# mims-harvard/SubGNN

Hardware: AMD Instinct MI355X
Metric: subgraphs/sec fwd+bwd (all 3 channels on) + achieved HBM GB/s (higher is better)
Workload: dtype f32; 1 GPU; synthetic DENSITY-style BA base graph n=1000000 m=10 (9998512 undirected edges), 50000 BFS subgraphs x 20 nodes per GPU (weak form; BASELINE configs[3] "50k sharded across 8" as worded is --scaling strong), all_density hparams (N 10/43, P 57/183, S 42, 1 layer), D=64, full pass = sampling + similarities + fwd + bwd + Adam; subgraphs_per_gpu=50000, subgraphs_total=50000

## Files before the change

### include/subgnn_hip.h

```cpp
#ifndef SUBGNN_HIP_H
#define SUBGNN_HIP_H

#include <stdint.h>

#ifdef __cplusplus
extern "C" {
#endif

#define SGNN_OK                  0
#define SGNN_ERR_BAD_ARG        -1
#define SGNN_ERR_SET_TOO_LARGE  -2
#define SGNN_ERR_NNZ_TOO_LARGE  -3
#define SGNN_ERR_LAUNCH         -4
#define SGNN_ERR_UNSUPPORTED_D  -5

#define SGNN_ABI_VERSION 12
int sgnn_abi_version(void);
int sgnn_warm_up(void* stream);
const char* sgnn_last_error(void);

int sgnn_degree_sequence(const int64_t* rowptr, const int32_t* col, int64_t nnz,
                         const int32_t* full_degree, const uint8_t* self_loops,
                         const int64_t* set_ptr, const int32_t* set_nodes, int64_t n_sets,
                         int64_t max_set_size, int sorted,
// ... 103 lines not shown
                          void* stream);
int sgnn_triangular_walks_both(const int64_t* rowptr, const int32_t* col, const int32_t* col_sorted, int64_t nnz,
                               const int64_t* patch_ptr, const int32_t* patch_nodes, const int64_t* inb_ptr,
                               const int32_t* inb_nodes, int64_t n_items, int64_t walks_per_patch, int64_t walk_len,
                               double beta, uint64_t seed, uint64_t stream_id_int, uint64_t stream_id_bor,
                               int64_t item_base, int64_t max_id, int64_t* out, void* stream);

int sgnn_patch_in_border(const int64_t* rowptr, const int32_t* col, int64_t nnz,
                         const int32_t* node_order, const int32_t* node_pos, int64_t n_nodes,
                         const int64_t* patch_ptr, const int32_t* patch_nodes, int64_t n_patches,
                         uint8_t* out_flag, void* stream);
int64_t sgnn_patch_in_border_huge_workspace_bytes(int64_t total_nodes);
int sgnn_patch_in_border_huge(const int64_t* rowptr, const int32_t* col, int64_t nnz,
                              const int32_t* node_order, const int32_t* node_pos, int64_t n_nodes,
                              const int64_t* patch_ptr, const int32_t* patch_nodes, int64_t n_patches,
                              int64_t total_nodes, uint8_t* out_flag, void* workspace, int64_t workspace_bytes,
                              void* stream);

int sgnn_sp_similarity_dense(const double* apsp, int64_t n_cols,
                             const int64_t* set_ptr, const int32_t* set_nodes, int64_t n_sets,
                             float* out, void* stream);
int64_t sgnn_bfs_hops_workspace_bytes(int64_t max_id, int64_t n_sources, int max_hops);
int sgnn_bfs_hops(const int64_t* rowptr, const int32_t* col, int64_t nnz, int64_t max_id,
                  const int32_t* sources, int64_t n_sources, int max_hops, int node_major, int pull_alpha,
                  uint8_t* dist, void* workspace, int64_t workspace_bytes, void* stream);
int sgnn_min_hops_to_sets(const uint8_t* dist, int64_t n_sources, int64_t max_id, int node_major,
                          const int64_t* set_ptr, const int32_t* set_nodes, int64_t n_sets,
                          float* out, void* stream);
int64_t sgnn_bfs_min_hops_workspace_bytes(int64_t max_id, int64_t n_sources, int max_hops, int64_t n_sets);
int sgnn_bfs_min_hops_to_sets(const int64_t* rowptr, const int32_t* col, int64_t nnz, int64_t max_id,
                              const int32_t* sources, int64_t n_sources, int max_hops, int pull_alpha, int push_levels,
                              const int64_t* set_ptr, const int32_t* set_nodes, int64_t n_sets,
                              float* out, int32_t* out_status, void* workspace, int64_t workspace_bytes, void* stream);

int sgnn_dtw_order_keys(const int64_t* x_ptr, const int32_t* x_val, int64_t n_x, int64_t* out_keys, void* stream);
int64_t sgnn_dtw_workspace_bytes(int64_t n_x, int64_t max_x_len, int64_t n_y, int64_t max_y_len);
int sgnn_dtw_similarity(const int64_t* x_ptr, const int32_t* x_val, int64_t n_x, int64_t max_x_len,
                        const int64_t* y_ptr, const int32_t* y_val, int64_t n_y, int64_t max_y_len,
                        int tie_order, int kernel, const int32_t* x_order, float* out, void* workspace,
                        int64_t workspace_bytes, void* stream);
int sgnn_dtw_similarity_live(const int64_t* x_ptr, const int32_t* x_val, int64_t n_x, int64_t max_x_len,
                             const int64_t* y_ptr, const int32_t* y_val, int64_t n_y, int64_t max_y_len,
                             int tie_order, int kernel, const int32_t* x_order, const int64_t* x_live_range, float* out,
                             void* workspace, int64_t workspace_bytes, void* stream);

int64_t sgnn_dtw_exact_workspace_bytes(int64_t n_x, int64_t max_x_len, int64_t n_y, int64_t max_y_len);
int sgnn_dtw_exact_similarity(const int64_t* x_ptr, const int32_t* x_val, int64_t n_x, int64_t max_x_len,
                              const int64_t* y_ptr, const int32_t* y_val, int64_t n_y, int64_t max_y_len,
                              int kernel, const int32_t* x_order, float* out, void* workspace,
                              int64_t workspace_bytes, void* stream);
int sgnn_dtw_exact_similarity_live(const int64_t* x_ptr, const int32_t* x_val, int64_t n_x, int64_t max_x_len,
                                   const int64_t* y_ptr, const int32_t* y_val, int64_t n_y, int64_t max_y_len,
                                   int kernel, const int32_t* x_order, const int64_t* x_live_range, float* out,
                                   void* workspace, int64_t workspace_bytes, void* stream);

int sgnn_cc_embed_fwd(const float* E, int64_t D,
                      const int64_t* set_ptr, const int32_t* set_nodes, int64_t n_sets,
                      int aggregator, int64_t padded_len, float* out, int32_t* out_arg, void* stream);
int sgnn_cc_embed_fwd_f16(const uint16_t* E_half, int64_t D,
                          const int64_t* set_ptr, const int32_t* set_nodes, int64_t n_sets,
                          int aggregator, int64_t padded_len, float* out, int32_t* out_arg, void* stream);
int sgnn_cc_embed_bwd(const float* grad_out, int64_t D,
                      const int64_t* set_ptr, const int32_t* set_nodes, int64_t n_sets,
                      int aggregator, const int32_t* arg, float* grad_E, void* stream);

#define SGNN_SRC_DENSE  0
// ... 219 lines not shown
```

### subgnn_amd/_lib.py

```python
import ctypes
import os

_HERE = os.path.dirname(os.path.abspath(__file__))
LIB_PATH = os.path.join(_HERE, 'lib', 'libsubgnn_hip.so')

c_i64 = ctypes.c_int64
c_u64 = ctypes.c_uint64
c_int = ctypes.c_int
c_dbl = ctypes.c_double
c_ptr = ctypes.c_void_p


class MpnArgs(ctypes.Structure):
    _fields_ = [('src', ctypes.c_int32), ('sims_per_edge', ctypes.c_int32),
                ('R', c_i64), ('A', c_i64), ('D', c_i64),
                ('x', c_ptr), ('ids', c_ptr), ('id_div', c_i64), ('edge_mask', c_ptr), ('row_mask', c_ptr),
                ('sims', c_ptr), ('sims_ld', c_i64), ('sim_col', c_ptr), ('wp', c_ptr), ('bp', c_ptr),
                ('x_f16', ctypes.c_int32), ('z_act', c_ptr), ('flags', ctypes.c_int32)]


SIGNATURES = {
    'sgnn_abi_version': (c_int, []),
    'sgnn_warm_up': (c_int, [c_ptr]),
    'sgnn_last_error': (ctypes.c_char_p, []),
# ... 15 lines not shown
    'sgnn_cc_compact_huge': (c_int, [c_ptr, c_ptr, c_ptr, c_i64, c_i64, c_int, c_i64, c_i64, c_ptr, c_ptr, c_ptr, c_ptr, c_i64, c_ptr]),
    'sgnn_subgraph_properties_workspace_bytes': (c_i64, [c_i64]),
    'sgnn_subgraph_properties': (c_int, [c_ptr, c_ptr, c_i64, c_i64, c_int, c_ptr, c_ptr, c_i64, c_i64, c_i64, c_ptr, c_ptr, c_ptr, c_i64,
                                         c_ptr]),
    'sgnn_patch_in_border_huge_workspace_bytes': (c_i64, [c_i64]),
    'sgnn_patch_in_border_huge': (c_int, [c_ptr, c_ptr, c_i64, c_ptr, c_ptr, c_i64, c_ptr, c_ptr, c_i64, c_i64, c_ptr, c_ptr, c_i64, c_ptr]),
    'sgnn_sort_sets': (c_int, [c_ptr, c_ptr, c_i64, c_i64, c_ptr, c_ptr, c_ptr]),
    'sgnn_khop_border_workspace_bytes': (c_i64, [c_i64, c_i64, c_int]),
    'sgnn_khop_border_bitmap_fits_lds': (c_int, [c_i64]),
    'sgnn_khop_border': (c_int, [c_ptr, c_ptr, c_i64, c_i64, c_ptr, c_ptr, c_i64, c_int, c_int, c_ptr, c_ptr, c_ptr,
                                 c_ptr, c_ptr, c_i64, c_int, c_ptr]),
    'sgnn_khop_border_arena': (c_int, [c_ptr, c_ptr, c_i64, c_i64, c_ptr, c_ptr, c_i64, c_int, c_ptr, c_ptr, c_ptr, c_ptr,
                                       c_i64, c_int, c_ptr]),
    'sgnn_khop_border_sample_workspace_bytes': (c_i64, [c_i64, c_i64, c_int, c_int, c_int]),
    'sgnn_khop_border_sample': (c_int, [c_ptr, c_ptr, c_ptr, c_i64, c_i64, c_ptr, c_ptr, c_i64, c_int, c_i64, c_u64, c_u64, c_i64,
                                        c_ptr, c_ptr, c_ptr, c_ptr, c_ptr, c_ptr, c_i64, c_int, c_ptr]),
    'sgnn_khop1_border_sorted': (c_int, [c_ptr, c_ptr, c_ptr, c_i64, c_i64, c_ptr, c_ptr, c_i64, c_ptr, c_ptr, c_ptr, c_ptr, c_i64,
                                         c_int, c_ptr]),
    'sgnn_sample_border_anchors': (c_int, [c_ptr, c_ptr, c_ptr, c_i64, c_ptr, c_i64, c_u64, c_u64, c_i64, c_int, c_ptr, c_ptr,
                                           c_ptr]),
    'sgnn_sample_anchors_padded': (c_int, [c_ptr, c_i64, c_i64, c_i64, c_u64, c_u64, c_ptr, c_ptr]),
    'sgnn_sample_anchors_ragged': (c_int, [c_ptr, c_ptr, c_i64, c_ptr, c_i64, c_u64, c_u64, c_i64, c_ptr, c_ptr]),
    'sgnn_choice_ragged': (c_int, [c_ptr, c_ptr, c_i64, c_i64, c_u64, c_u64, c_i64, c_ptr, c_ptr]),
    'sgnn_triangular_walks_both': (c_int, [c_ptr, c_ptr, c_ptr, c_i64, c_ptr, c_ptr, c_ptr, c_ptr, c_i64, c_i64, c_i64, c_dbl, c_u64,
                                           c_u64, c_u64, c_i64, c_i64, c_ptr, c_ptr]),
    'sgnn_triangular_walks': (c_int, [c_ptr, c_ptr, c_ptr, c_i64, c_ptr, c_i64, c_ptr, c_ptr, c_ptr, c_ptr, c_int,
                                      c_i64, c_i64, c_i64, c_dbl, c_u64, c_u64, c_i64, c_i64, c_int, c_ptr, c_ptr]),
    'sgnn_patch_in_border': (c_int, [c_ptr, c_ptr, c_i64, c_ptr, c_ptr, c_i64, c_ptr, c_ptr, c_i64, c_ptr, c_ptr]),
    'sgnn_sp_similarity_dense': (c_int, [c_ptr, c_i64, c_ptr, c_ptr, c_i64, c_ptr, c_ptr]),
    'sgnn_bfs_hops_workspace_bytes': (c_i64, [c_i64, c_i64, c_int]),
    'sgnn_bfs_min_hops_workspace_bytes': (c_i64, [c_i64, c_i64, c_int, c_i64]),
    'sgnn_bfs_min_hops_to_sets': (c_int, [c_ptr, c_ptr, c_i64, c_i64, c_ptr, c_i64, c_int, c_int, c_int, c_ptr, c_ptr, c_i64, c_ptr, c_ptr,
                                          c_ptr, c_i64, c_ptr]),
    'sgnn_bfs_hops': (c_int, [c_ptr, c_ptr, c_i64, c_i64, c_ptr, c_i64, c_int, c_int, c_int, c_ptr, c_ptr, c_i64, c_ptr]),
    'sgnn_min_hops_to_sets': (c_int, [c_ptr, c_i64, c_i64, c_int, c_ptr, c_ptr, c_i64, c_ptr, c_ptr]),
    'sgnn_dtw_workspace_bytes': (c_i64, [c_i64, c_i64, c_i64, c_i64]),
    'sgnn_dtw_similarity': (c_int, [c_ptr, c_ptr, c_i64, c_i64, c_ptr, c_ptr, c_i64, c_i64, c_int, c_int, c_ptr, c_ptr, c_ptr,
                                    c_i64, c_ptr]),
    'sgnn_dtw_order_keys': (c_int, [c_ptr, c_ptr, c_i64, c_ptr, c_ptr]),
    'sgnn_dtw_similarity_live': (c_int, [c_ptr, c_ptr, c_i64, c_i64, c_ptr, c_ptr, c_i64, c_i64, c_int, c_int, c_ptr, c_ptr, c_ptr,
                                         c_ptr, c_i64, c_ptr]),
    'sgnn_dtw_exact_workspace_bytes': (c_i64, [c_i64, c_i64, c_i64, c_i64]),
    'sgnn_dtw_exact_similarity': (c_int, [c_ptr, c_ptr, c_i64, c_i64, c_ptr, c_ptr, c_i64, c_i64, c_int, c_ptr, c_ptr, c_ptr,
                                          c_i64, c_ptr]),
    'sgnn_dtw_exact_similarity_live': (c_int, [c_ptr, c_ptr, c_i64, c_i64, c_ptr, c_ptr, c_i64, c_i64, c_int, c_ptr, c_ptr, c_ptr,
                                               c_ptr, c_i64, c_ptr]),
    'sgnn_cc_embed_fwd': (c_int, [c_ptr, c_i64, c_ptr, c_ptr, c_i64, c_int, c_i64, c_ptr, c_ptr, c_ptr]),
    'sgnn_cc_embed_bwd': (c_int, [c_ptr, c_i64, c_ptr, c_ptr, c_i64, c_int, c_ptr, c_ptr, c_ptr]),
    'sgnn_mpn_fwd_chunks': (c_int, [ctypes.POINTER(MpnArgs)]),
    'sgnn_mpn_fwd': (c_int, [ctypes.POINTER(MpnArgs), c_ptr, c_ptr, c_ptr]),
    'sgnn_mpn_fwd_many_max_bodies': (c_i64, []),
    'sgnn_mpn_fwd_many': (c_int, [c_i64, c_ptr, c_ptr, c_ptr, c_ptr]),
    'sgnn_mpn_bwd': (c_int, [ctypes.POINTER(MpnArgs), c_ptr, c_ptr, c_ptr, c_ptr, c_ptr]),
    'sgnn_attn_scores_epilogue': (c_int, [c_ptr, c_ptr, c_ptr, c_i64, c_i64, c_i64, c_ptr, c_ptr]),
    'sgnn_attn_scores_f16_workspace_bytes': (c_i64, [c_i64]),
    'sgnn_attn_scores_fwd_f16': (c_int, [c_ptr, c_ptr, c_ptr, c_ptr, c_i64, c_i64, c_i64, c_ptr, c_ptr, c_i64, c_ptr]),
    'sgnn_lstm_supported': (c_int, [c_i64]),
    'sgnn_lstm_fwd': (c_int, [c_ptr, c_ptr, c_ptr, c_ptr, c_ptr, c_i64, c_i64, c_i64, c_ptr, c_ptr, c_ptr, c_ptr, c_ptr]),
    'sgnn_lstm_bwd': (c_int, [c_ptr, c_ptr, c_ptr, c_ptr, c_ptr, c_i64, c_i64, c_i64, c_ptr, c_ptr]),
    'sgnn_masked_sum_fwd': (c_int, [c_ptr, c_ptr, c_i64, c_i64, c_i64, c_ptr, c_ptr]),
    'sgnn_masked_sum_bwd': (c_int, [c_ptr, c_ptr, c_i64, c_i64, c_i64, c_ptr, c_ptr]),
    'sgnn_masked_sum_slot_fwd': (c_int, [c_ptr, c_ptr, c_i64, c_i64, c_i64, c_ptr, c_i64, c_ptr]),
    'sgnn_masked_sum_slot_bwd': (c_int, [c_ptr, c_i64, c_ptr, c_i64, c_i64, c_i64, c_ptr, c_ptr]),
    'sgnn_masked_sum_slots_fwd': (c_int, [c_ptr, c_ptr, c_ptr, c_i64, c_ptr, c_i64, c_i64, c_ptr, c_i64, c_ptr]),
    'sgnn_masked_sum_slots_bwd': (c_int, [c_ptr, c_i64, c_ptr, c_i64, c_i64, c_ptr, c_ptr, c_ptr, c_i64, c_ptr]),
    'sgnn_readout_sum_fwd': (c_int, [c_ptr, c_i64, c_ptr, c_ptr, c_ptr, c_ptr, c_i64, c_i64, c_i64, c_ptr, c_i64, c_ptr]),
# ... 126 lines not shown
```

### subgnn_amd/csrc/similarity.hip

```cpp
#include "common.h"
#include <type_traits>

__global__ __launch_bounds__(256) void sp_similarity_dense_kernel(
    const double* __restrict__ apsp, int64_t n_cols,
    const int64_t* __restrict__ set_ptr, const int32_t* __restrict__ set_nodes,
    float* __restrict__ out)
{
    const int64_t r = blockIdx.y;
    const int64_t beg = set_ptr[r];
    const int n = (int)(set_ptr[r + 1] - beg);
    for (int64_t c = blockIdx.x * (int64_t)blockDim.x + threadIdx.x; c < n_cols; c += (int64_t)gridDim.x * blockDim.x) {
        float res = 0.f;
        if (n > 0) {
            double m = apsp[(int64_t)(set_nodes[beg] - 1) * n_cols + c];
            for (int i = 1; i < n; ++i) {
                const double v = apsp[(int64_t)(set_nodes[beg + i] - 1) * n_cols + c];
                m = v < m ? v : m;
            }
            res = (float)m;
        }
        out[r * n_cols + c] = res;
    }
}

// ... 528 lines not shown
    for (int l = 2; l <= last_level && flags[l - 1] != 0; ++l) {
        bool pl, ppl;
        int kk;
        msbfs_mode(fvol, pull_above, push_levels, l, pl, ppl, kk);
        n_written += pl ? 1 : 0;
    }
    const uint64_t* lcur = pull ? B[(k + 1) % 3] : frontier;
    const uint64_t* lold = pull ? B[k % 3] : nullptr;
    for (int64_t t = blockIdx.x * (int64_t)blockDim.x + threadIdx.x; t < total; t += (int64_t)gridDim.x * blockDim.x) {
        if (reduce_last)
            msbfs_set_reduce_item(lcur, n_words, n_sources, set_ptr, set_nodes, set_seen, out, last_level, rs, t, lold);
        const int64_t r = t / n_words, w = t % n_words;
        uint64_t all = ~0ull;
        for (int64_t i = set_ptr[r]; i < set_ptr[r + 1]; ++i) {
            const int64_t v = set_nodes[i];
            if (!fdone[v]) all &= B[n_written % 3][v * rs + w];
        }
        uint64_t missing = ~all;
        while (missing) {
            const int b = __ffsll((unsigned long long)missing) - 1;
            missing &= missing - 1;
            const int64_t s = w * 64 + b;
            if (s < n_sources) out[r * n_sources + s] = 0.f;
        }
    }
}

__global__ void msbfs_status_kernel(const int32_t* __restrict__ flags, int max_hops, int32_t* __restrict__ status,
                                    const unsigned long long* __restrict__ fvol, unsigned long long pull_above, int push_levels)
{
    if (threadIdx.x == 0 && blockIdx.x == 0) msbfs_write_status(flags, fvol, pull_above, push_levels, max_hops, status);
}

static int msbfs_run(const int64_t* rowptr, const int32_t* col, int64_t nnz, int64_t max_id,
                     const int32_t* sources, int64_t n_sources, int max_hops, int node_major, uint8_t* dist,
                     const int64_t* set_ptr, const int32_t* set_nodes, int64_t n_sets, float* set_out,
                     void* workspace, hipStream_t st, int pull_alpha, int32_t* status = nullptr, int push_levels = -1)
{
    if (push_levels < 0 || pull_alpha == 0 || push_levels > max_hops) push_levels = max_hops;
    if (push_levels < 1) push_levels = 1;
    const int g_bfs_alpha = pull_alpha < 0 ? MSBFS_DEFAULT_ALPHA : pull_alpha;
    const int64_t n_ids = max_id + 1;
    const int64_t n_words = (n_sources + 63) / 64;
    const int64_t ss = node_major ? 1 : n_ids, sv = node_major ? n_sources : 1;
    const int64_t rs = msbfs_row_stride(n_words);
    uint64_t* seen = (uint64_t*)workspace;
    uint64_t* frontier = seen + n_ids * rs;
    uint64_t* next = frontier + n_ids * rs;
    unsigned long long* fvol = (unsigned long long*)(next + n_ids * rs);
    int32_t* flags = (int32_t*)(fvol + max_hops + 2);
    uint32_t* fbits = (uint32_t*)(((uintptr_t)(flags + max_hops + 2) + 7) & ~(uintptr_t)7);
    const int64_t fwords = (n_ids + 31) / 32;
    uint8_t* fdone = (uint8_t*)(fbits + 2 * fwords);
    uint64_t* set_seen = (uint64_t*)(((uintptr_t)(fbits + 2 * fwords + (n_ids + 3) / 4) + 7) & ~(uintptr_t)7);
    const unsigned long long pull_above =
        g_bfs_alpha > 0 ? (unsigned long long)((nnz * n_words) / g_bfs_alpha) : ~0ull;
    const int big = sgnn_grid_for(n_ids * ((dist && n_sources > rs) ? n_sources : rs), 256);
    hipLaunchKernelGGL(msbfs_init_kernel, dim3(big), dim3(256), 0, st, sources, n_sources, n_words, n_ids, seen,
                       frontier, next, dist, flags, fvol, fbits, max_hops, rs, set_seen, set_out ? n_sets * n_words : 0,
                       set_out, set_out ? n_sets * n_sources : 0);
    SGNN_CHECK_LAUNCH();
    hipLaunchKernelGGL(msbfs_seed_kernel, dim3((int)((n_sources + 255) / 256)), dim3(256), 0, st, sources, n_sources,
                       n_words, n_ids, seen, frontier, dist, ss, sv, fbits, rs);
    SGNN_CHECK_LAUNCH();
    const int g_sets = set_out ? sgnn_grid_for(n_sets * n_words, 256) : 0;
    MsbfsSets sets;
    sets.set_ptr = set_ptr; sets.set_nodes = set_nodes; sets.n_sets = set_out ? n_sets : 0; sets.set_seen = set_seen; sets.out = set_out;
    const int g_expand = sgnn_grid_for(n_ids * 16, 256);
    const int g_commit = sgnn_grid_for(n_ids, 256, 256 * 4);
    MsbfsBufs bufs;
    bufs.b[0] = seen; bufs.b[1] = next; bufs.b[2] = frontier;
    for (int level = 1; level <= max_hops; ++level) {
        hipLaunchKernelGGL(msbfs_level_kernel, dim3(g_expand), dim3(256), 0, st, rowptr, col, n_ids, n_words, n_sources,
                           bufs, flags, fvol, pull_above, push_levels, level, fbits, fbits + fwords, fdone, rs, sets, dist, ss, sv);
        SGNN_CHECK_LAUNCH();
        if (level <= push_levels) {
            hipLaunchKernelGGL(msbfs_commit_kernel, dim3(g_commit), dim3(256), 0, st, rowptr, n_ids, n_words, n_sources, seen,
                               frontier, next, dist, flags, fvol, level, ss, sv, fbits, fdone, rs, pull_above, push_levels);
            SGNN_CHECK_LAUNCH();
        }
    }
    if (set_out) {
        hipLaunchKernelGGL(msbfs_set_finalize_kernel, dim3(g_sets), dim3(256), 0, st, seen, n_words, n_sources, set_ptr,
                           set_nodes, n_sets, set_out, rs, frontier, set_seen, flags, max_hops, status, next, fvol, pull_above,
                           push_levels, fdone);
        SGNN_CHECK_LAUNCH();
    }
    if (status && !set_out) {
        hipLaunchKernelGGL(msbfs_status_kernel, dim3(1), dim3(64), 0, st, flags, max_hops, status, fvol, pull_above, push_levels);
        SGNN_CHECK_LAUNCH();
    }
    return SGNN_OK;
}

extern "C" int sgnn_bfs_hops(const int64_t* rowptr, const int32_t* col, int64_t nnz, int64_t max_id,
                             const int32_t* sources, int64_t n_sources, int max_hops, int node_major, int pull_alpha,
                             uint8_t* dist, void* workspace, int64_t workspace_bytes, void* stream)
{
    if (!rowptr || !col || !sources || !dist || !workspace || n_sources < 0 || max_hops < 1 || max_hops > 254)
        return SGNN_ERR_BAD_ARG;
    if (nnz >= (1ll << 31)) return SGNN_ERR_NNZ_TOO_LARGE;
    if (workspace_bytes < sgnn_bfs_hops_workspace_bytes(max_id, n_sources, max_hops)) return SGNN_ERR_BAD_ARG;
    if (n_sources == 0) return SGNN_OK;
    return msbfs_run(rowptr, col, nnz, max_id, sources, n_sources, max_hops, node_major, dist, nullptr, nullptr, 0,
                     nullptr, workspace, (hipStream_t)stream, pull_alpha);
}

extern "C" int64_t sgnn_bfs_min_hops_workspace_bytes(int64_t max_id, int64_t n_sources, int max_hops, int64_t n_sets) {
    const int64_t n_words = (n_sources + 63) / 64;
    return sgnn_bfs_hops_workspace_bytes(max_id, n_sources, max_hops) + 16 + n_sets * n_words * 8;
}

extern "C" int sgnn_bfs_min_hops_to_sets(const int64_t* rowptr, const int32_t* col, int64_t nnz, int64_t max_id,
                                         const int32_t* sources, int64_t n_sources, int max_hops, int pull_alpha, int push_levels,
                                         const int64_t* set_ptr, const int32_t* set_nodes, int64_t n_sets,
                                         float* out, int32_t* out_status, void* workspace, int64_t workspace_bytes,
                                         void* stream)
{
    if (!rowptr || !col || !sources || !set_ptr || !set_nodes || !out || !workspace || n_sources < 0 || n_sets < 0 ||
        max_hops < 1 || max_hops > 254)
        return SGNN_ERR_BAD_ARG;
    if (nnz >= (1ll << 31)) return SGNN_ERR_NNZ_TOO_LARGE;
    if (workspace_bytes < sgnn_bfs_min_hops_workspace_bytes(max_id, n_sources, max_hops, n_sets)) return SGNN_ERR_BAD_ARG;
    if (n_sources == 0 || n_sets == 0) return SGNN_OK;
    return msbfs_run(rowptr, col, nnz, max_id, sources, n_sources, max_hops, 0, nullptr, set_ptr, set_nodes, n_sets, out,
                     workspace, (hipStream_t)stream, pull_alpha, out_status, push_levels);
}

__global__ void min_hops_to_sets_kernel(const uint8_t* __restrict__ dist, int64_t n_sources, int64_t n_ids,
                                        const int64_t* __restrict__ set_ptr, const int32_t* __restrict__ set_nodes,
                                        int64_t n_sets, float* __restrict__ out, int64_t ss, int64_t sv)
{
    const int64_t total = n_sets * n_sources;
    for (int64_t t = blockIdx.x * (int64_t)blockDim.x + threadIdx.x; t < total; t += (int64_t)gridDim.x * blockDim.x) {
        const int64_t r = t / n_sources, a = t % n_sources;
        const int64_t beg = set_ptr[r];
        const int n = (int)(set_ptr[r + 1] - beg);
        int m = 0;
        for (int i = 0; i < n; ++i) {
            int d = dist[a * ss + (int64_t)set_nodes[beg + i] * sv];
            if (d == 255) d = 0;
            m = (i == 0 || d < m) ? d : m;
        }
        out[t] = (float)m;
    }
}

extern "C" int sgnn_min_hops_to_sets(const uint8_t* dist, int64_t n_sources, int64_t max_id, int node_major,
                                     const int64_t* set_ptr, const int32_t* set_nodes, int64_t n_sets,
                                     float* out, void* stream)
{
    if (!dist || !set_ptr || !set_nodes || !out || n_sources < 0 || n_sets < 0) return SGNN_ERR_BAD_ARG;
    if (n_sets * n_sources == 0) return SGNN_OK;
    hipLaunchKernelGGL(min_hops_to_sets_kernel, dim3(sgnn_grid_for(n_sets * n_sources, 256)), dim3(256), 0,
                       (hipStream_t)stream, dist, n_sources, max_id + 1, set_ptr, set_nodes, n_sets, out,
                       node_major ? 1 : max_id + 1, node_major ? n_sources : 1);
    SGNN_CHECK_LAUNCH();
    return SGNN_OK;
}
// ... 3 lines not shown
```

### subgnn_amd/hotpath.py

```python
import time

import collections

import torch

from . import ops, tape, gamma, subgraph_utils
from .graph_step import record, recording_key
from . import anchor_patch_samplers as aps

MAX_PINT_BYTES = 16 << 30


class StageTimer:

    def __init__(self, enabled=True):
        self.enabled, self.marks, self.host = enabled, [], []

    def mark(self, name):
        if self.enabled:
            e = torch.cuda.Event(enable_timing=True)
            e.record()
            self.marks.append((name, e))
            self.host.append(time.perf_counter())

# ... 7 lines not shown
        return out


def _hand_over(stream, *objs):
    for o in objs:
        if o is None:
            continue
        if isinstance(o, torch.Tensor):
            if o.is_cuda:
                o.record_stream(stream)
            for nm in ('_sgnn_ids32', '_sgnn_sorted', '_sgnn_both', '_sgnn_all', '_sgnn_mask', '_sgnn_mask_u8'):
                extra = getattr(o, nm, None)
                if extra is not None:
                    _hand_over(stream, extra)
        elif isinstance(o, ops.Ragged):
            _hand_over(stream, o.ptr, o.nodes)
        elif isinstance(o, dict):
            _hand_over(stream, *o.values())
        elif isinstance(o, (list, tuple)):
            _hand_over(stream, *o)


BFS_LEVEL_MARGIN = 2
WALKS_ON_SIDE_MAX_SETS = 16384


def _bfs_levels(model, key, max_hops):
    hint = model.__dict__.setdefault('_bfs_level_hint', {})
    k = hint.get(key)
    return max_hops if k is None else min(max_hops, k + BFS_LEVEL_MARGIN + 1)


BFS_PUSH_MARGIN = 1


def _bfs_push_levels(model, key):
    k = model.__dict__.setdefault('_bfs_push_hint', {}).get(key)
    return -1 if not k else int(k) - 1 + BFS_PUSH_MARGIN


def _bfs_note(model, st, key, status, max_hops, enqueued, redo):
    hint = model.__dict__.setdefault('_bfs_level_hint', {})
    if torch.cuda.is_current_stream_capturing():
        if hint.get(key) is None:
            raise RuntimeError('a recorded pass needs the BFS depth of an earlier eager pass (GraphedPasses warms up first)')
        pool = model.__dict__.setdefault('_bfs_status_pool', [])
        if not pool:
            raise RuntimeError('no pinned status buffer left for a recorded search: GraphedPasses._record provides them')
        host = pool.pop()
        host.copy_(status, non_blocking=True)
        st.bfs_checks.append((key, host, None, max_hops, enqueued, None))
        return
    if hint.get(key) is None:
        last, more, first_pull = status.tolist()[:3]
        model.__dict__.setdefault('_bfs_push_hint', {})[key] = first_pull
        if more:
            raise RuntimeError('position-channel BFS: level %d still reached new nodes -- hparams["max_bfs_hops"] = %d '
                               'is smaller than the depth of this graph from the anchors' % (max_hops, max_hops))
        hint[key] = last
        return
    pool = model.__dict__.setdefault('_bfs_status_pool', [])
    host = pool.pop() if pool else torch.empty(4, dtype=torch.int32).pin_memory()
    host.copy_(status, non_blocking=True)
    ev = torch.cuda.Event()
    ev.record(torch.cuda.current_stream())
    st.bfs_checks.append((key, host, ev, max_hops, enqueued, redo))
# ... 202 lines not shown
    sims = {}
    a_sets = ai = ae = None
    det = bool(getattr(model, '_deterministic', ops.DETERMINISTIC))
    side.wait_stream(main)
    with torch.cuda.stream(side):
        new_patches = hp['use_structure'] and pool is None and (split != 'test' or getattr(model, 'structure_anchors', None) is None)
        structure_anchors = getattr(model, 'structure_anchors', None) if pool is None else pool['structure_anchors']
        if new_patches:
            if shard is not None and shard.deal_shared and hp['structure_patch_type'] == 'triangular_random_walk':
                n_p = hp['max_sim_epochs'] * hp['n_anchor_patches_structure'] * hp['n_layers']
                structure_anchors = _deal_rows(shard, n_p, lambda lo, hi: aps.sample_structure_anchor_patches(
                    hp, g, dev, hp['max_sim_epochs'], trim=False, share=(lo, hi)), (hp['sample_walk_len'],), torch.int64, dev,
                    key=('S_patches', split))
                st.attrs['structure_anchors'] = structure_anchors
            else:
                structure_anchors = st.attrs['structure_anchors'] = aps.sample_structure_anchor_patches(hp, g, dev, hp['max_sim_epochs'], trim=False)
            if side is main:
                t.mark('S_patches_walks')
        patch_ev = None
        if hp['use_structure'] and side is not main:
            patch_ev = torch.cuda.Event()
            patch_ev.record(side)
        def position_block():
            if hp['use_position']:
                anchors_pos_ext = getattr(model, 'anchors_pos_ext', None)
                if anchors_pos_ext is None or split != 'test':
                    anchors_pos_ext = st.attrs['anchors_pos_ext'] = aps.init_anchors_pos_ext(hp, g, dev, epoch=ep)
                    if det:
                        for v in anchors_pos_ext.values():
                            ops.presort_ids(v, g.max_id)
                pint = {l: ops.choice_ragged(subs, hp['n_anchor_patches_pos_in'], seed,
                                             tape.stream_id(tape.STREAM_P_INT, split, l, ep), item_base=base) for l in range(L)}
                st.per_split['anchors_pos_int'] = pint
                for l in range(L):
                    if shard is not None and shard.deal_shared:
                        cap = hp.get('max_bfs_hops', 32)
                        if getattr(shard, 'emulator', None) is not None:
                            w, status = _emulated_position_sims(g, anchors_pos_ext[l], cc_sets, cc_ids, shard, cap, (split, l))
                        else:
                            w, status = _dealt_position_sims(g, anchors_pos_ext[l], cc_sets, cc_ids, shard, cap)
                        w = w.view(S, C, -1)
                        model.__dict__.setdefault('_bfs_level_hint', {}).setdefault(('P_out_dealt', split, l), 0)
                        _bfs_note(model, st, ('P_out_dealt', split, l), status, cap, cap, None)
                    else:
                        cap = hp.get('max_bfs_hops', 32)
                        nlev = _bfs_levels(model, ('P_out', split, l), cap)
                        src = anchors_pos_ext[l].to(torch.int32).contiguous()
                        w, status = ops.bfs_min_hops_to_sets(g, src, cc_sets, max_hops=nlev, want_status=True,
                                                             push_levels=_bfs_push_levels(model, ('P_out', split, l)))

                        def redo(levels, src=src, l=l, sims=sims):
                            _hand_over(torch.cuda.current_stream(), src, cc_sets)
                            w2, st2 = ops.bfs_min_hops_to_sets(g, src, cc_sets, max_hops=levels, want_status=True)
                            sims[('P', 'out', l)] = w2.view(S, C, -1).contiguous()
                            return st2.tolist()
                        _bfs_note(model, st, ('P_out', split, l), status, cap, nlev, redo)
                        w = w.view(S, C, -1)
                    sims[('P', 'out', l)] = w.contiguous()
                    if C == 1:
                        sims[('P', 'in', l)] = ops.ZeroSims((S, C, hp['n_anchor_patches_pos_in']), dev)
                    else:
                        uniq, inv = torch.unique(pint[l], return_inverse=True)
                        if uniq.numel() * (g.max_id + 1) <= MAX_PINT_BYTES:
                            d = ops.bfs_hops(g, uniq.to(torch.int32).contiguous(), max_hops=hp.get('max_bfs_hops', 32),
                                             node_major=True)
                            full = ops.min_hops_to_sets(d, cc_sets, node_major=True).view(S, C, -1)
                            w = torch.gather(full, 2, inv.view(S, 1, -1).expand(S, C, -1))
                        else:
                            w = _pint_sims_streamed(g, uniq, inv, cc_sets, S, C, hp.get('max_bfs_hops', 32))
                        sims[('P', 'in', l)] = (w * real.unsqueeze(-1)).contiguous()
                if side is main:
                    t.mark('P_bfs_sims')
        late_bfs = bool(hp.get('bfs_beside_dtw', False)) and side is not main and hp['use_structure'] and hp['use_position'] \
            and not defer_dtw and not (shard is not None and shard.deal_shared)
        wos = hp.get('walks_on_side_stream')
        walks_on_side = (bool(wos) if wos is not None else cc_sets.n <= WALKS_ON_SIDE_MAX_SETS) and side is not main and hp['use_structure']

        def structure_walks(degree_sequences=True):
            nonlocal a_sets, ai, ae
            if new_patches and shard is not None and shard.deal_shared:
                W_, T_ = hp['n_triangular_walks'], hp['random_walk_len']

                def both(lo, hi):
                    mine = structure_anchors[lo:hi].contiguous()
                    v = aps.patch_node_views(mine)
                    iw, bw = aps.perform_random_walks_both(hp, g, mine, v, first_patch=lo)
# ... 528 lines not shown
```

### subgnn_amd/ops.py

```python
import collections
import ctypes
import functools
import threading

import numpy as np
import torch

from . import _lib
from ._lib import MpnArgs, check

PAD = 0


def _ptr(t):
    return None if t is None else ctypes.c_void_p(t.data_ptr())


_RAW_STREAM = getattr(torch._C, '_cuda_getCurrentRawStream', None)
_CUR_DEVICE = getattr(torch._C, '_cuda_getDevice', None)


def _stream():
    if _RAW_STREAM is not None and _CUR_DEVICE is not None:
        return ctypes.c_void_p(_RAW_STREAM(_CUR_DEVICE()))
# ... 199 lines not shown
            hubs = torch.nonzero(deg >= thr).view(-1)
            H = int(hubs.numel())
            W, rows_n = (H + 31) // 32, self.max_id + 1
            if 0 < H and rows_n * W * 4 <= self.HUB_BITMAP_BYTES:
                dev = self.device
                hub_index = torch.full((self.max_id + 1,), -1, dtype=torch.int32, device=dev)
                hub_index[hubs] = torch.arange(H, dtype=torch.int32, device=dev)
                hdeg = deg[hubs]
                owner = torch.repeat_interleave(torch.arange(H, dtype=torch.int64, device=dev), hdeg)
                start = torch.cumsum(hdeg, 0) - hdeg
                pos = torch.arange(owner.numel(), dtype=torch.int64, device=dev) - start[owner] + self.rowptr[hubs][owner]
                x = self.col_sorted[pos].to(torch.int64)
                words = torch.zeros(rows_n * W, dtype=torch.int64, device=dev)
                words.index_add_(0, x * W + (owner >> 5), torch.ones_like(owner) << (owner & 31))
                out = (hub_index, words.to(torch.int32).view(rows_n, W).contiguous(), W)
        self.__dict__['_hub_tables'] = out
        return out

    def node_records(self):
        cached = self.__dict__.get('_node_records', False)
        if cached is not False:
            return cached
        out = None
        hub = self.hub_tables()
        if hub is not None:
            deg = (self.rowptr[1:] - self.rowptr[:-1]).to(torch.int32)
            sl = self.self_loops.to(torch.int32)
            z = ((sl.to(torch.int64) << 24) | torch.where(hub[0] >= 0, hub[0], torch.full_like(hub[0], 0xffffff)).to(torch.int64)).to(torch.int32)
            full = self.full_degree if self.full_degree is not None else deg + sl
            out = torch.stack([self.rowptr[:-1].to(torch.int32), deg, z, full.to(torch.int32)], 1).contiguous()
        self.__dict__['_node_records'] = out
        return out


_WARM = set()


def warm_up(device=None):
    if not torch.cuda.is_available():
        return 0.0
    dev = torch.device('cuda', torch.cuda.current_device()) if device is None else torch.device(device)
    if dev.type != 'cuda' or str(dev) in _WARM:
        return 0.0
    import time
    t0 = time.perf_counter()
    _WARM.add(str(dev))
    with torch.cuda.device(dev), torch.random.fork_rng(devices=[dev]):
        check(_lib.load().sgnn_warm_up(_stream()), 'sgnn_warm_up')
        i64 = torch.arange(8, device=dev)
        i32 = i64.to(torch.int32)
        f32 = torch.rand(8, 8, device=dev, requires_grad=True)
        torch.cumsum(i64, 0); torch.sort(i64); torch.argsort(i32); i64.index_select(0, i64 % 4); i64.max(); (i64 != 0).sum()
        torch.zeros(9, dtype=torch.int64, device=dev).scatter_(0, i64, i64); torch.where(i64 > 3, i64, i64 - 1)
        torch.unique(i64 % 3, return_inverse=True); torch.repeat_interleave(i64, 2); torch.stack((i64.sum(), i64.sum()))
        w = torch.rand(8, 8, device=dev, requires_grad=True)
        b = torch.rand(8, device=dev, requires_grad=True)
        y = torch.nn.functional.dropout(torch.relu(torch.nn.functional.linear(f32, w, b)), 0.1, True)
        y = y + torch.addmm(b, f32, w.t()) + torch.bmm(f32.view(2, 4, 8), w.view(2, 8, 4).transpose(1, 2).contiguous().transpose(1, 2)).reshape(8, 4).sum() \
            + (f32 @ b).view(-1, 1) + torch.cat([f32, w], 0)[:8]
        y.sum().backward()
        torch._foreach_norm([w.grad, b.grad])
        torch.cuda.synchronize(dev)
    return time.perf_counter() - t0



# ... 432 lines not shown
    return out


def sp_similarity_dense(apsp, sets):
    lib = _lib.load()
    _req(apsp, torch.float64, 'apsp')
    n_cols = apsp.shape[1]
    out = torch.empty((sets.n, n_cols), dtype=torch.float32, device=apsp.device)
    check(lib.sgnn_sp_similarity_dense(_ptr(apsp), n_cols, _ptr(sets.ptr), _ptr(sets.nodes), sets.n, _ptr(out),
                                       _stream()), 'sgnn_sp_similarity_dense')
    return out


def probe_stream_copy(src, dst, bytes_per_lane):
    nbytes = src.numel() * src.element_size()
    assert dst.numel() * dst.element_size() == nbytes and src.is_cuda and dst.is_cuda
    check(_lib.load().sgnn_probe_stream_copy(_ptr(src), _ptr(dst), nbytes, int(bytes_per_lane), _stream()),
          'sgnn_probe_stream_copy')


def bfs_hops(g, sources, max_hops=64, node_major=False, pull_alpha=-1):
    lib = _lib.load()
    _req(sources, torch.int32, 'sources')
    ns = sources.numel()
    shape = (g.max_id + 1, ns) if node_major else (ns, g.max_id + 1)
    dist = torch.empty(shape, dtype=torch.uint8, device=g.device)
    wsb = lib.sgnn_bfs_hops_workspace_bytes(g.max_id, ns, max_hops)
    ws = torch.empty(wsb // 8 + 1, dtype=torch.int64, device=g.device)
    check(lib.sgnn_bfs_hops(_ptr(g.rowptr), _ptr(g.col), g.nnz, g.max_id, _ptr(sources), ns, max_hops,
                            1 if node_major else 0, int(pull_alpha), _ptr(dist), _ptr(ws), wsb, _stream()), 'sgnn_bfs_hops')
    return dist


def bfs_min_hops_to_sets(g, sources, sets, max_hops=64, want_status=False, pull_alpha=-1, push_levels=-1):
    lib = _lib.load()
    _req(sources, torch.int32, 'sources')
    ns = sources.numel()
    out = torch.empty((sets.n, ns), dtype=torch.float32, device=g.device)
    status = torch.zeros(4, dtype=torch.int32, device=g.device) if want_status else None
    wsb = lib.sgnn_bfs_min_hops_workspace_bytes(g.max_id, ns, max_hops, sets.n)
    ws = torch.empty(wsb // 8 + 1, dtype=torch.int64, device=g.device)
    check(lib.sgnn_bfs_min_hops_to_sets(_ptr(g.rowptr), _ptr(g.col), g.nnz, g.max_id, _ptr(sources), ns, max_hops,
                                        int(pull_alpha), int(push_levels), _ptr(sets.ptr), _ptr(sets.nodes), sets.n, _ptr(out), _ptr(status), _ptr(ws), wsb,
                                        _stream()), 'sgnn_bfs_min_hops_to_sets')
    return (out, status) if want_status else out


def min_hops_to_sets(dist, sets, node_major=False):
    lib = _lib.load()
    _req(dist, torch.uint8, 'dist')
    if node_major:
        n_ids, ns = dist.shape
    else:
        ns, n_ids = dist.shape
    out = torch.empty((sets.n, ns), dtype=torch.float32, device=dist.device)
    check(lib.sgnn_min_hops_to_sets(_ptr(dist), ns, n_ids - 1, 1 if node_major else 0, _ptr(sets.ptr), _ptr(sets.nodes),
                                    sets.n, _ptr(out), _stream()), 'sgnn_min_hops_to_sets')
    return out


_HASH_COEF = {}


def _row_representatives(rows):
    n, w = rows.shape
    dev = rows.device
    coef = _HASH_COEF.get((w, dev))
    if coef is None:
        g = torch.Generator(device='cpu').manual_seed(0x5DEECE66D)
        coef = _HASH_COEF[(w, dev)] = (torch.randint(-(1 << 62), 1 << 62, (w,), generator=g, dtype=torch.int64) | 1).to(dev)
    h = (rows.to(torch.int64) * coef).sum(dim=1)
    hs, perm = torch.sort(h)
# ... 1952 lines not shown
```

Measured before the change: 6.734 million subgraphs/s.

## Stop multi-source BFS once every reachable subgraph set has been reached

Adds a connected-component labelling pass (union-find hooking with host-polled convergence, cached per graph) and a new BFS-to-sets variant. The variant computes, per set and source word, which sources share the set's component, and sets a device flag that halts further levels once every such pair has been reached. This avoids expanding BFS frontiers over the rest of the graph after all set distances are known. Position hops now default to this 'sets' mode. The cost is an extra reduction kernel per level and a one-time component pass that synchronises with the host each round.

```diff
diff --git a/include/subgnn_hip.h b/include/subgnn_hip.h
--- a/include/subgnn_hip.h
+++ b/include/subgnn_hip.h
@@ -159,6 +159,15 @@
                               const int32_t* sources, int64_t n_sources, int max_hops, int pull_alpha, int push_levels,
                               const int64_t* set_ptr, const int32_t* set_nodes, int64_t n_sets,
                               float* out, int32_t* out_status, void* workspace, int64_t workspace_bytes, void* stream);
+int64_t sgnn_graph_component_labels_workspace_bytes(int64_t max_id);
+int sgnn_graph_component_labels(const int64_t* rowptr, const int32_t* col, int64_t nnz, int64_t max_id,
+                                int32_t* labels, void* workspace, int64_t workspace_bytes, void* stream);
+int64_t sgnn_bfs_min_hops_closing_workspace_bytes(int64_t max_id, int64_t n_sources, int max_hops, int64_t n_sets);
+int sgnn_bfs_min_hops_to_sets_closing(const int64_t* rowptr, const int32_t* col, int64_t nnz, int64_t max_id,
+                                      const int32_t* sources, int64_t n_sources, int max_hops, int pull_alpha, int push_levels,
+                                      const int32_t* labels, const int64_t* set_ptr, const int32_t* set_nodes,
+                                      int64_t n_sets, float* out, int32_t* out_status, void* workspace, int64_t workspace_bytes,
+                                      void* stream);
 
 int sgnn_dtw_order_keys(const int64_t* x_ptr, const int32_t* x_val, int64_t n_x, int64_t* out_keys, void* stream);
 int64_t sgnn_dtw_workspace_bytes(int64_t n_x, int64_t max_x_len, int64_t n_y, int64_t max_y_len);
diff --git a/subgnn_amd/_lib.py b/subgnn_amd/_lib.py
--- a/subgnn_amd/_lib.py
+++ b/subgnn_amd/_lib.py
@@ -71,6 +71,11 @@
     'sgnn_bfs_min_hops_workspace_bytes': (c_i64, [c_i64, c_i64, c_int, c_i64]),
     'sgnn_bfs_min_hops_to_sets': (c_int, [c_ptr, c_ptr, c_i64, c_i64, c_ptr, c_i64, c_int, c_int, c_int, c_ptr, c_ptr, c_i64, c_ptr, c_ptr,
                                           c_ptr, c_i64, c_ptr]),
+    'sgnn_graph_component_labels_workspace_bytes': (c_i64, [c_i64]),
+    'sgnn_graph_component_labels': (c_int, [c_ptr, c_ptr, c_i64, c_i64, c_ptr, c_ptr, c_i64, c_ptr]),
+    'sgnn_bfs_min_hops_closing_workspace_bytes': (c_i64, [c_i64, c_i64, c_int, c_i64]),
+    'sgnn_bfs_min_hops_to_sets_closing': (c_int, [c_ptr, c_ptr, c_i64, c_i64, c_ptr, c_i64, c_int, c_int, c_int, c_ptr, c_ptr,
+                                                  c_ptr, c_i64, c_ptr, c_ptr, c_ptr, c_i64, c_ptr]),
     'sgnn_bfs_hops': (c_int, [c_ptr, c_ptr, c_i64, c_i64, c_ptr, c_i64, c_int, c_int, c_int, c_ptr, c_ptr, c_i64, c_ptr]),
     'sgnn_min_hops_to_sets': (c_int, [c_ptr, c_i64, c_i64, c_int, c_ptr, c_ptr, c_i64, c_ptr, c_ptr]),
     'sgnn_dtw_workspace_bytes': (c_i64, [c_i64, c_i64, c_i64, c_i64]),
diff --git a/subgnn_amd/csrc/similarity.hip b/subgnn_amd/csrc/similarity.hip
--- a/subgnn_amd/csrc/similarity.hip
+++ b/subgnn_amd/csrc/similarity.hip
@@ -584,10 +584,116 @@
     if (threadIdx.x == 0 && blockIdx.x == 0) msbfs_write_status(flags, fvol, pull_above, push_levels, max_hops, status);
 }
 
+struct MsbfsClosing {
+    const int32_t* labels;
+    const int32_t* sources;
+    uint64_t* wanted;
+    uint32_t* open;
+    uint32_t* ticket;
+    uint32_t* closed;
+};
+
+#define MSBFS_CLOSING_LDS_SOURCES 1024
+
+__global__ __launch_bounds__(256) void msbfs_closing_reduce_kernel(
+    MsbfsBufs B, int64_t n_words, int64_t n_sources, int64_t rs, MsbfsSets sets, MsbfsClosing c, int32_t* __restrict__ flags,
+    const unsigned long long* __restrict__ fvol, unsigned long long pull_above, int push_levels, int level)
+{
+    if (level > 0 && flags[level - 1] == 0) return;
+    __shared__ int32_t s_lab[MSBFS_CLOSING_LDS_SOURCES];
+    const bool lds = n_sources <= MSBFS_CLOSING_LDS_SOURCES;
+    const uint64_t* cur = B.b[2];
+    const uint64_t* old = nullptr;
+    if (level > 0) {
+        bool pull, prev_pull;
+        int k;
+        msbfs_mode(fvol, pull_above, push_levels, level, pull, prev_pull, k);
+        if (pull) { cur = B.b[(k + 1) % 3]; old = B.b[k % 3]; }
+    } else if (lds) {
+        for (int64_t i = threadIdx.x; i < n_sources; i += blockDim.x) s_lab[i] = c.labels[c.sources[i]];
+        __syncthreads();
+    }
+    bool open = false;
+    const int64_t total = sets.n_sets * n_words;
+    for (int64_t t = blockIdx.x * (int64_t)blockDim.x + threadIdx.x; t < total; t += (int64_t)gridDim.x * blockDim.x) {
+        const int64_t r = t / n_words, w = t % n_words;
+        const int64_t beg = sets.set_ptr[r], end = sets.set_ptr[r + 1];
+        uint64_t want = 0;
+        if (level == 0) {
+            bool one = end > beg;
+            int32_t common = -1;
+            for (int64_t i = beg; i < end; ++i) {
+                const int32_t lab = c.labels[sets.set_nodes[i]];
+                if (i == beg) common = lab; else if (lab != common) one = false;
+            }
+            if (one)
+                for (int b = 0; b < 64 && w * 64 + b < n_sources; ++b) {
+                    const int64_t s = w * 64 + b;
+                    if ((lds ? s_lab[s] : c.labels[c.sources[s]]) == common) want |= 1ull << b;
+                }
+            c.wanted[t] = want;
+        } else
+            want = c.wanted[t];
+        const uint64_t have = sets.set_seen[t];
+        if ((want & ~have) == 0) continue;
+        uint64_t acc = 0;
+        for (int64_t i = beg; i < end; ++i) {
+            const int64_t o = (int64_t)sets.set_nodes[i] * rs + w;
+            acc |= old ? (cur[o] & ~old[o]) : cur[o];
+        }
+        const uint64_t fresh = acc & want & ~have;
+        if (fresh) {
+            sets.set_seen[t] = have | fresh;
+            uint64_t bits = fresh;
+            while (bits) {
+                const int b = __ffsll((unsigned long long)bits) - 1;
+                bits &= bits - 1;
+                sets.out[r * n_sources + w * 64 + b] = (float)level;
+            }
+        }
+        if (want & ~(have | fresh)) open = true;
+    }
+    if (__syncthreads_or(open ? 1 : 0) && threadIdx.x == 0) atomicOr(&c.open[level], 1u);
+    if (threadIdx.x == 0) {
+        __threadfence();
+        if (atomicAdd(&c.ticket[level], 1u) == gridDim.x - 1) {
+            __threadfence();
+            if (__hip_atomic_load(&c.open[level], __ATOMIC_ACQUIRE, __HIP_MEMORY_SCOPE_AGENT) == 0) {
+                c.closed[0] = (uint32_t)level + 1;
+                flags[level] = 0;
+            }
+        }
+    }
+}
+
+__global__ void msbfs_closing_status_kernel(const int32_t* __restrict__ flags, const unsigned long long* __restrict__ fvol,
+                                            unsigned long long pull_above, int push_levels, int max_hops,
+                                            const uint32_t* __restrict__ closed, int32_t* __restrict__ status)
+{
+    if (threadIdx.x != 0 || blockIdx.x != 0) return;
+    const int c = (int)closed[0];
+    int last = c ? c - 1 : 0;
+    if (!c) for (int l = 1; l <= max_hops; ++l) if (flags[l]) last = l;
+    status[0] = last;
+    status[1] = !c && flags[max_hops] != 0;
+    int first_pull = 0;
+    for (int l = 2; l <= (c ? last : last + 1) && l <= max_hops && first_pull == 0; ++l) {
+        bool pull, prev_pull;
+        int k;
+        msbfs_mode(fvol, pull_above, push_levels, l, pull, prev_pull, k);
+        if (pull) first_pull = l;
+    }
+    status[2] = first_pull;
+    status[3] = 0;
+}
+
+static inline int64_t msbfs_closing_state_words(int max_hops) { return (2 * ((int64_t)max_hops + 2) + 2 + 1) / 2; }
+
 static int msbfs_run(const int64_t* rowptr, const int32_t* col, int64_t nnz, int64_t max_id,
                      const int32_t* sources, int64_t n_sources, int max_hops, int node_major, uint8_t* dist,
                      const int64_t* set_ptr, const int32_t* set_nodes, int64_t n_sets, float* set_out,
-                     void* workspace, hipStream_t st, int pull_alpha, int32_t* status = nullptr, int push_levels = -1)
+                     void* workspace, hipStream_t st, int pull_alpha, int32_t* status = nullptr, int push_levels = -1,
+                     const int32_t* labels = nullptr)
 {
     if (push_levels < 0 || pull_alpha == 0 || push_levels > max_hops) push_levels = max_hops;
     if (push_levels < 1) push_levels = 1;
@@ -608,8 +714,18 @@
     const unsigned long long pull_above =
         g_bfs_alpha > 0 ? (unsigned long long)((nnz * n_words) / g_bfs_alpha) : ~0ull;
     const int big = sgnn_grid_for(n_ids * ((dist && n_sources > rs) ? n_sources : rs), 256);
+    MsbfsClosing cl = {};
+    int64_t n_zero = set_out ? n_sets * n_words : 0;
+    if (labels) {
+        cl.labels = labels; cl.sources = sources;
+        cl.open = (uint32_t*)(set_seen + n_sets * n_words);
+        cl.ticket = cl.open + max_hops + 2;
+        cl.closed = cl.ticket + max_hops + 2;
+        cl.wanted = set_seen + n_sets * n_words + msbfs_closing_state_words(max_hops);
+        n_zero += msbfs_closing_state_words(max_hops);
+    }
     hipLaunchKernelGGL(msbfs_init_kernel, dim3(big), dim3(256), 0, st, sources, n_sources, n_words, n_ids, seen,
-                       frontier, next, dist, flags, fvol, fbits, max_hops, rs, set_seen, set_out ? n_sets * n_words : 0,
+                       frontier, next, dist, flags, fvol, fbits, max_hops, rs, set_seen, n_zero,
                        set_out, set_out ? n_sets * n_sources : 0);
     SGNN_CHECK_LAUNCH();
     hipLaunchKernelGGL(msbfs_seed_kernel, dim3((int)((n_sources + 255) / 256)), dim3(256), 0, st, sources, n_sources,
@@ -622,6 +738,31 @@
     const int g_commit = sgnn_grid_for(n_ids, 256, 256 * 4);
     MsbfsBufs bufs;
     bufs.b[0] = seen; bufs.b[1] = next; bufs.b[2] = frontier;
+    if (labels) {
+        MsbfsSets none = sets;
+        none.n_sets = 0;
+        for (int level = 0; level <= max_hops; ++level) {
+            if (level >= 1) {
+                hipLaunchKernelGGL(msbfs_level_kernel, dim3(g_expand), dim3(256), 0, st, rowptr, col, n_ids, n_words, n_sources,
+                                   bufs, flags, fvol, pull_above, push_levels, level, fbits, fbits + fwords, fdone, rs, none, dist, ss, sv);
+                SGNN_CHECK_LAUNCH();
+            }
+            if (level >= 1 && level <= push_levels) {
+                hipLaunchKernelGGL(msbfs_commit_kernel, dim3(g_commit), dim3(256), 0, st, rowptr, n_ids, n_words, n_sources, seen,
+                                   frontier, next, dist, flags, fvol, level, ss, sv, fbits, fdone, rs, pull_above, push_levels);
+                SGNN_CHECK_LAUNCH();
+            }
+            hipLaunchKernelGGL(msbfs_closing_reduce_kernel, dim3(g_sets), dim3(256), 0, st, bufs, n_words, n_sources, rs, sets, cl,
+                               flags, fvol, pull_above, push_levels, level);
+            SGNN_CHECK_LAUNCH();
+        }
+        if (status) {
+            hipLaunchKernelGGL(msbfs_closing_status_kernel, dim3(1), dim3(64), 0, st, flags, fvol, pull_above, push_levels, max_hops,
+                               cl.closed, status);
+            SGNN_CHECK_LAUNCH();
+        }
+        return SGNN_OK;
+    }
     for (int level = 1; level <= max_hops; ++level) {
         hipLaunchKernelGGL(msbfs_level_kernel, dim3(g_expand), dim3(256), 0, st, rowptr, col, n_ids, n_words, n_sources,
                            bufs, flags, fvol, pull_above, push_levels, level, fbits, fbits + fwords, fdone, rs, sets, dist, ss, sv);
@@ -677,6 +818,98 @@
     if (n_sources == 0 || n_sets == 0) return SGNN_OK;
     return msbfs_run(rowptr, col, nnz, max_id, sources, n_sources, max_hops, 0, nullptr, set_ptr, set_nodes, n_sets, out,
                      workspace, (hipStream_t)stream, pull_alpha, out_status, push_levels);
+}
+
+extern "C" int64_t sgnn_bfs_min_hops_closing_workspace_bytes(int64_t max_id, int64_t n_sources, int max_hops, int64_t n_sets) {
+    const int64_t n_words = (n_sources + 63) / 64;
+    return sgnn_bfs_min_hops_workspace_bytes(max_id, n_sources, max_hops, n_sets) +
+           8 * (msbfs_closing_state_words(max_hops) + n_sets * n_words);
+}
+
+extern "C" int sgnn_bfs_min_hops_to_sets_closing(const int64_t* rowptr, const int32_t* col, int64_t nnz, int64_t max_id,
+                                                 const int32_t* sources, int64_t n_sources, int max_hops, int pull_alpha,
+                                                 int push_levels, const int32_t* labels, const int64_t* set_ptr,
+                                                 const int32_t* set_nodes, int64_t n_sets, float* out, int32_t* out_status,
+                                                 void* workspace, int64_t workspace_bytes, void* stream)
+{
+    if (!rowptr || !col || !sources || !labels || !set_ptr || !set_nodes || !out || !workspace || n_sources < 0 || n_sets < 0 ||
+        max_hops < 1 || max_hops > 254)
+        return SGNN_ERR_BAD_ARG;
+    if (nnz >= (1ll << 31)) return SGNN_ERR_NNZ_TOO_LARGE;
+    if (workspace_bytes < sgnn_bfs_min_hops_closing_workspace_bytes(max_id, n_sources, max_hops, n_sets)) return SGNN_ERR_BAD_ARG;
+    if (n_sources == 0 || n_sets == 0) return SGNN_OK;
+    return msbfs_run(rowptr, col, nnz, max_id, sources, n_sources, max_hops, 0, nullptr, set_ptr, set_nodes, n_sets, out,
+                     workspace, (hipStream_t)stream, pull_alpha, out_status, push_levels, labels);
+}
+
+__device__ __forceinline__ int32_t cc_graph_root(const int32_t* lab, int32_t x)
+{
+    for (int32_t p = __hip_atomic_load(&lab[x], __ATOMIC_RELAXED, __HIP_MEMORY_SCOPE_AGENT); p != x;
+         p = __hip_atomic_load(&lab[x], __ATOMIC_RELAXED, __HIP_MEMORY_SCOPE_AGENT))
+        x = p;
+    return x;
+}
+
+__global__ void cc_graph_init_kernel(int32_t* __restrict__ lab, int64_t n_ids)
+{
+    for (int64_t v = blockIdx.x * (int64_t)blockDim.x + threadIdx.x; v < n_ids; v += (int64_t)gridDim.x * blockDim.x) lab[v] = (int32_t)v;
+}
+
+__global__ __launch_bounds__(256) void cc_graph_hook_kernel(const int64_t* __restrict__ rowptr, const int32_t* __restrict__ col,
+                                                            int64_t n_ids, int32_t* lab, int32_t* __restrict__ changed)
+{
+    const int sub = threadIdx.x & 15;
+    const int64_t group = blockIdx.x * (int64_t)(blockDim.x >> 4) + (threadIdx.x >> 4);
+    const int64_t n_groups = (int64_t)gridDim.x * (blockDim.x >> 4);
+    bool any = false;
+    for (int64_t v = group; v < n_ids; v += n_groups) {
+        const int64_t r0 = rowptr[v], r1 = rowptr[v + 1];
+        for (int64_t e = r0 + sub; e < r1; e += 16) {
+            const int32_t u = col[e];
+            if (u < 0 || u >= n_ids || u == v) continue;
+            const int32_t a = cc_graph_root(lab, (int32_t)v), b = cc_graph_root(lab, u);
+            if (a != b) {
+                atomicMin(&lab[a > b ? a : b], a > b ? b : a);
+                any = true;
+            }
+        }
+    }
+    if (any) *changed = 1;
+}
+
+__global__ void cc_graph_flatten_kernel(int32_t* lab, int64_t n_ids)
+{
+    for (int64_t v = blockIdx.x * (int64_t)blockDim.x + threadIdx.x; v < n_ids; v += (int64_t)gridDim.x * blockDim.x) {
+        const int32_t r = cc_graph_root(lab, (int32_t)v);
+        if (r != (int32_t)v) __hip_atomic_store(&lab[v], r, __ATOMIC_RELAXED, __HIP_MEMORY_SCOPE_AGENT);
+    }
+}
+
+extern "C" int64_t sgnn_graph_component_labels_workspace_bytes(int64_t max_id) { (void)max_id; return 16; }
+
+extern "C" int sgnn_graph_component_labels(const int64_t* rowptr, const int32_t* col, int64_t nnz, int64_t max_id,
+                                           int32_t* labels, void* workspace, int64_t workspace_bytes, void* stream)
+{
+    if (!rowptr || (!col && nnz > 0) || !labels || !workspace || max_id < 0 || nnz < 0 ||
+        workspace_bytes < sgnn_graph_component_labels_workspace_bytes(max_id))
+        return SGNN_ERR_BAD_ARG;
+    hipStream_t st = (hipStream_t)stream;
+    const int64_t n_ids = max_id + 1;
+    int32_t* changed = (int32_t*)workspace;
+    hipLaunchKernelGGL(cc_graph_init_kernel, dim3(sgnn_grid_for(n_ids, 256)), dim3(256), 0, st, labels, n_ids);
+    SGNN_CHECK_LAUNCH();
+    for (int64_t round = 0; round <= n_ids; ++round) {
+        int32_t host = 0;
+        if (hipMemsetAsync(changed, 0, 4, st) != hipSuccess) return SGNN_ERR_LAUNCH;
+        hipLaunchKernelGGL(cc_graph_hook_kernel, dim3(sgnn_grid_for(n_ids * 16, 256)), dim3(256), 0, st, rowptr, col, n_ids, labels, changed);
+        SGNN_CHECK_LAUNCH();
+        hipLaunchKernelGGL(cc_graph_flatten_kernel, dim3(sgnn_grid_for(n_ids, 256)), dim3(256), 0, st, labels, n_ids);
+        SGNN_CHECK_LAUNCH();
+        if (hipMemcpyAsync(&host, changed, 4, hipMemcpyDeviceToHost, st) != hipSuccess || hipStreamSynchronize(st) != hipSuccess)
+            return SGNN_ERR_LAUNCH;
+        if (!host) break;
+    }
+    return SGNN_OK;
 }
 
 __global__ void min_hops_to_sets_kernel(const uint8_t* __restrict__ dist, int64_t n_sources, int64_t n_ids,
diff --git a/subgnn_amd/hotpath.py b/subgnn_amd/hotpath.py
--- a/subgnn_amd/hotpath.py
+++ b/subgnn_amd/hotpath.py
@@ -63,6 +63,13 @@
 
 
 BFS_PUSH_MARGIN = 1
+
+
+def _position_until(hp):
+    until = hp.get('position_search_until', 'sets')
+    if until not in ('sets', 'nodes'):
+        raise ValueError("hparams['position_search_until'] must be 'sets' or 'nodes', not %r" % (until,))
+    return until
 
 
 def _bfs_push_levels(model, key):
@@ -331,6 +338,7 @@
                 pint = {l: ops.choice_ragged(subs, hp['n_anchor_patches_pos_in'], seed,
                                              tape.stream_id(tape.STREAM_P_INT, split, l, ep), item_base=base) for l in range(L)}
                 st.per_split['anchors_pos_int'] = pint
+                until = _position_until(hp)
                 for l in range(L):
                     if shard is not None and shard.deal_shared:
                         cap = hp.get('max_bfs_hops', 32)
@@ -346,11 +354,11 @@
                         nlev = _bfs_levels(model, ('P_out', split, l), cap)
                         src = anchors_pos_ext[l].to(torch.int32).contiguous()
                         w, status = ops.bfs_min_hops_to_sets(g, src, cc_sets, max_hops=nlev, want_status=True,
-                                                             push_levels=_bfs_push_levels(model, ('P_out', split, l)))
-
-                        def redo(levels, src=src, l=l, sims=sims):
+                                                             push_levels=_bfs_push_levels(model, ('P_out', split, l)), until=until)
+
+                        def redo(levels, src=src, l=l, sims=sims, until=until):
                             _hand_over(torch.cuda.current_stream(), src, cc_sets)
-                            w2, st2 = ops.bfs_min_hops_to_sets(g, src, cc_sets, max_hops=levels, want_status=True)
+                            w2, st2 = ops.bfs_min_hops_to_sets(g, src, cc_sets, max_hops=levels, want_status=True, until=until)
                             sims[('P', 'out', l)] = w2.view(S, C, -1).contiguous()
                             return st2.tolist()
                         _bfs_note(model, st, ('P_out', split, l), status, cap, nlev, redo)
diff --git a/subgnn_amd/ops.py b/subgnn_amd/ops.py
--- a/subgnn_amd/ops.py
+++ b/subgnn_amd/ops.py
@@ -255,6 +255,21 @@
         self.__dict__['_node_records'] = out
         return out
 
+    def component_labels(self):
+        cached = self.__dict__.get('_component_labels')
+        if cached is None:
+            if torch.cuda.is_current_stream_capturing():
+                raise RuntimeError('DeviceGraph.component_labels() reads a word back per round and cannot be built while a stream '
+                                   'is capturing: call it (or run one eager search with until=\'sets\') before recording')
+            lib = _lib.load()
+            cached = torch.empty(self.max_id + 1, dtype=torch.int32, device=self.device)
+            wsb = lib.sgnn_graph_component_labels_workspace_bytes(self.max_id)
+            ws = torch.empty(wsb // 8 + 1, dtype=torch.int64, device=self.device)
+            check(lib.sgnn_graph_component_labels(_ptr(self.rowptr), _ptr(self.col), self.nnz, self.max_id, _ptr(cached), _ptr(ws),
+                                                  wsb, _stream()), 'sgnn_graph_component_labels')
+            self.__dict__['_component_labels'] = cached
+        return cached
+
 
 _WARM = set()
 
@@ -753,12 +768,23 @@
     return dist
 
 
-def bfs_min_hops_to_sets(g, sources, sets, max_hops=64, want_status=False, pull_alpha=-1, push_levels=-1):
+def bfs_min_hops_to_sets(g, sources, sets, max_hops=64, want_status=False, pull_alpha=-1, push_levels=-1, until='nodes'):
     lib = _lib.load()
     _req(sources, torch.int32, 'sources')
     ns = sources.numel()
     out = torch.empty((sets.n, ns), dtype=torch.float32, device=g.device)
     status = torch.zeros(4, dtype=torch.int32, device=g.device) if want_status else None
+    if until == 'sets':
+        labels = g.component_labels()
+        wsb = lib.sgnn_bfs_min_hops_closing_workspace_bytes(g.max_id, ns, max_hops, sets.n)
+        ws = torch.empty(wsb // 8 + 1, dtype=torch.int64, device=g.device)
+        check(lib.sgnn_bfs_min_hops_to_sets_closing(_ptr(g.rowptr), _ptr(g.col), g.nnz, g.max_id, _ptr(sources), ns, max_hops,
+                                                    int(pull_alpha), int(push_levels), _ptr(labels), _ptr(sets.ptr),
+                                                    _ptr(sets.nodes), sets.n, _ptr(out), _ptr(status), _ptr(ws), wsb, _stream()),
+              'sgnn_bfs_min_hops_to_sets_closing')
+        return (out, status) if want_status else out
+    if until != 'nodes':
+        raise ValueError("until must be 'nodes' or 'sets', not %r" % (until,))
     wsb = lib.sgnn_bfs_min_hops_workspace_bytes(g.max_id, ns, max_hops, sets.n)
     ws = torch.empty(wsb // 8 + 1, dtype=torch.int64, device=g.device)
     check(lib.sgnn_bfs_min_hops_to_sets(_ptr(g.rowptr), _ptr(g.col), g.nnz, g.max_id, _ptr(sources), ns, max_hops,
```

Measured after the change: 6.967 million subgraphs/s (median of 6 runs). 3.5% higher.
